# aanna0701/face-recognition-pytorch

Hardware: AMD Instinct MI355X
Metric: train imgs/sec IR-50-layout ResNet50 + ArcFace/PartialFC head, 112x112 (higher is better)
Workload: dtype bf16

## Files before the change

### face-recognition-pytorch_amd/frhip/csrc/bn.hip

```cpp
#include <cstdlib>
#include "common.h"
#include "frhip.h"

namespace frhip {

constexpr int EW_THREADS = 256;
#ifndef EW_UNROLL
#define EW_UNROLL 2
#endif
#ifndef EW_ROWS
#define EW_ROWS 16
#endif
constexpr int RED_GROUPS = 16;

template <typename T> struct EW {
    static constexpr int EPV = 16 / (int)sizeof(T);
};

template <typename T, bool BWD, bool RS = false>
__global__ __launch_bounds__(EW_THREADS) void colreduce_kernel(const T* __restrict__ x, const T* __restrict__ y,
                                                               const float* __restrict__ mean, const float* __restrict__ invstd,
                                                               const float* __restrict__ mscale, const float* __restrict__ mshift,
                                                               float* __restrict__ partial, int rows, int C,
                                                               const float* __restrict__ rowscale = nullptr, int rows_per = 1) {
// ... 116 lines not shown
                                   const float* __restrict__ gamma, const float* __restrict__ beta,
                                   float* __restrict__ running_mean, float* __restrict__ running_var,
                                   float momentum, float eps, float* __restrict__ mean_out,
                                   float* __restrict__ invstd_out, float* __restrict__ scale, float* __restrict__ shift) {
    __shared__ float red[FIN_MAX_PL][2][64];
    int c, pl;
    float s1, s2;
    if constexpr (SMALL) {
        c = blockIdx.x * 16 + (threadIdx.x & 15); pl = threadIdx.x >> 4;
        sum_parts16(parts, nparts, C, c, pl, reinterpret_cast<float (*)[2][16]>(&red[0][0][0]), s1, s2);
    } else {
        c = blockIdx.x * 64 + (threadIdx.x & 63); pl = threadIdx.x >> 6;
        sum_parts(parts, nparts, C, c, pl, red, s1, s2);
    }
    if (pl != 0 || c >= C) return;
    const float mu = s1 / count;
    float var = s2 / count - mu * mu;
    var = var < 0.f ? 0.f : var;
    const float is = rsqrtf(var + eps);
    mean_out[c] = mu; invstd_out[c] = is;
    const float sc = gamma[c] * is;
    scale[c] = sc; shift[c] = beta[c] - mu * sc;
    if (running_mean) {
        running_mean[c] = (1.f - momentum) * running_mean[c] + momentum * mu;
        const float unbiased = count > 1.f ? var * count / (count - 1.f) : var;
        running_var[c] = (1.f - momentum) * running_var[c] + momentum * unbiased;
    }
}

__global__ void bn_eval_kernel(int C, const float* __restrict__ gamma, const float* __restrict__ beta,
                               const float* __restrict__ rm, const float* __restrict__ rv, float eps,
                               float* __restrict__ scale, float* __restrict__ shift) {
    const int c = blockIdx.x * blockDim.x + threadIdx.x;
    if (c >= C) return;
    const float sc = gamma[c] * rsqrtf(rv[c] + eps);
    scale[c] = sc; shift[c] = beta[c] - rm[c] * sc;
}

template <bool SMALL>
__global__ __launch_bounds__(SMALL ? 256 : 1024) void bn_bwd_finalize_kernel(const float* __restrict__ parts, int nparts, int C, float count,
                                       const float* __restrict__ gamma, const float* __restrict__ mean,
                                       const float* __restrict__ invstd, float* __restrict__ dgamma,
                                       float* __restrict__ dbeta, float* __restrict__ ca, float* __restrict__ cb,
                                       float* __restrict__ cc) {
    __shared__ float red[FIN_MAX_PL][2][64];
    int c, pl;
    float s1, s2;
    if constexpr (SMALL) {
        c = blockIdx.x * 16 + (threadIdx.x & 15); pl = threadIdx.x >> 4;
        sum_parts16(parts, nparts, C, c, pl, reinterpret_cast<float (*)[2][16]>(&red[0][0][0]), s1, s2);
    } else {
        c = blockIdx.x * 64 + (threadIdx.x & 63); pl = threadIdx.x >> 6;
        sum_parts(parts, nparts, C, c, pl, red, s1, s2);
    }
    if (pl != 0 || c >= C) return;
    dgamma[c] += s2; dbeta[c] += s1;
    const float gi = gamma[c] * invstd[c], m2 = s2 / count, m1 = s1 / count;
    ca[c] = gi; cb[c] = -gi * invstd[c] * m2; cc[c] = gi * (mean[c] * invstd[c] * m2 - m1);
}

template <typename T, bool NT> __device__ __forceinline__ Vec16<T> ew_load(const T* p) {
    Vec16<T> r;
    if constexpr (NT) r.v = __builtin_nontemporal_load(reinterpret_cast<const decltype(r.v)*>(p));
    else r = *reinterpret_cast<const Vec16<T>*>(p);
    return r;
}
template <typename T, bool NT> __device__ __forceinline__ void ew_store(T* p, const Vec16<T>& x) {
    if constexpr (NT) __builtin_nontemporal_store(x.v, reinterpret_cast<decltype(x.v)*>(p));
    else *reinterpret_cast<Vec16<T>*>(p) = x;
}
static size_t EW_NT_BYTES = (size_t)(getenv("FRHIP_EW_NT_MB") ? atoi(getenv("FRHIP_EW_NT_MB")) : 0) << 20;
static int g_ew_nt = getenv("FRHIP_EW_NT") ? atoi(getenv("FRHIP_EW_NT")) : 1;

template <typename T, bool NTL, bool NTS, bool RS = false, bool INPLACE = false>
__global__ __launch_bounds__(EW_THREADS) void bn_apply_kernel(const T* __restrict__ y_in, const float* __restrict__ scale,
                                                              const float* __restrict__ shift, const T* __restrict__ res,
                                                              const float* __restrict__ rscale, const float* __restrict__ rshift,
                                                              int relu, T* __restrict__ out, int rows, int C,
                                                              const float* __restrict__ rowscale = nullptr, int rows_per = 1) {
    constexpr int EPV = EW<T>::EPV;
    const int vpr = C / EPV;
    const int cg = threadIdx.x % vpr, rl = threadIdx.x / vpr, rlanes = EW_THREADS / vpr;
    float sc[EPV], sh[EPV], rs[EPV], rb[EPV];
    const T* y = INPLACE ? out : y_in;
#pragma unroll
    for (int e = 0; e < EPV; ++e) {
        sc[e] = scale[cg * EPV + e]; sh[e] = shift[cg * EPV + e];
        rs[e] = rscale ? rscale[cg * EPV + e] : 1.f; rb[e] = rscale ? rshift[cg * EPV + e] : 0.f;
    }
#pragma unroll EW_UNROLL
    for (int r = blockIdx.x * rlanes + rl; r < rows; r += gridDim.x * rlanes) {
        const size_t idx = (size_t)r * C + cg * EPV;
        Vec16<T> a = ew_load<T, NTL>(y + idx);
        if constexpr (RS) {
            const float ks = rowscale[r / rows_per];
            Vec16<T> rv;
            if (res) rv = ew_load<T, NTL>(res + idx);
#pragma unroll
            for (int e = 0; e < EPV; ++e) {
                float o = (a.get(e) * sc[e] + sh[e]) * ks + (res ? rv.get(e) * rs[e] + rb[e] : 0.f);
                a.set(e, relu ? fmaxf(o, 0.f) : o);
            }
        } else if (res) {
            const Vec16<T> rv = ew_load<T, NTL>(res + idx);
#pragma unroll
            for (int e = 0; e < EPV; ++e) {
                float o = a.get(e) * sc[e] + sh[e] + (rv.get(e) * rs[e] + rb[e]);
                a.set(e, relu ? fmaxf(o, 0.f) : o);
            }
        } else {
#pragma unroll
            for (int e = 0; e < EPV; ++e) {
                float o = a.get(e) * sc[e] + sh[e];
                a.set(e, relu ? fmaxf(o, 0.f) : o);
            }
        }
        ew_store<T, NTS>(out + idx, a);
    }
}

template <typename T, bool NTL, bool NTS, bool RS = false>
__global__ __launch_bounds__(EW_THREADS) void bn_bwd_apply_kernel(const T* __restrict__ dout, const T* __restrict__ y,
                                                                  const float* __restrict__ ca, const float* __restrict__ cb,
                                                                  const float* __restrict__ cc, const float* __restrict__ mscale,
                                                                  const float* __restrict__ mshift, T* __restrict__ dy,
                                                                  int rows, int C, const float* __restrict__ rowscale = nullptr,
                                                                  int rows_per = 1) {
    constexpr int EPV = EW<T>::EPV;
    const int vpr = C / EPV;
    const int cg = threadIdx.x % vpr, rl = threadIdx.x / vpr, rlanes = EW_THREADS / vpr;
    float a_[EPV], b_[EPV], c_[EPV], ms[EPV], mb[EPV];
#pragma unroll
    for (int e = 0; e < EPV; ++e) {
        a_[e] = ca[cg * EPV + e]; b_[e] = cb[cg * EPV + e]; c_[e] = cc[cg * EPV + e];
        ms[e] = mscale ? mscale[cg * EPV + e] : 0.f; mb[e] = mscale ? mshift[cg * EPV + e] : 1.f;
    }
#pragma unroll EW_UNROLL
    for (int r = blockIdx.x * rlanes + rl; r < rows; r += gridDim.x * rlanes) {
        const size_t idx = (size_t)r * C + cg * EPV;
        const Vec16<T> d = ew_load<T, NTL>(dout + idx);
        Vec16<T> b = ew_load<T, NTL>(y + idx);
        float ks = 1.f;
        if constexpr (RS) ks = rowscale[r / rows_per];
#pragma unroll
        for (int e = 0; e < EPV; ++e) {
            const float yy = b.get(e);
            const float de = (yy * ms[e] + mb[e] > 0.f) ? d.get(e) * ks : 0.f;
            b.set(e, a_[e] * de + b_[e] * yy + c_[e]);
        }
        ew_store<T, NTS>(dy + idx, b);
    }
}

__global__ __launch_bounds__(256) void sum_partials_kernel(const float* __restrict__ partial, int nparts, int C, int which,
                                                           float* __restrict__ out) {
    __shared__ float red[16][16];
    const int cl = threadIdx.x & 15, pl = threadIdx.x >> 4;
    const int c = blockIdx.x * 16 + cl;
    float acc = 0.f;
    if (c < C) {
        int p = pl;
        for (; p + 7 * 16 < nparts; p += 8 * 16) {
            float v[8];
#pragma unroll
            for (int u = 0; u < 8; ++u) v[u] = partial[((size_t)(p + u * 16) * 2 + which) * C + c];
            acc += ((v[0] + v[1]) + (v[2] + v[3])) + ((v[4] + v[5]) + (v[6] + v[7]));
        }
        for (; p < nparts; p += 16) acc += partial[((size_t)p * 2 + which) * C + c];
    }
    red[pl][cl] = acc;
    __syncthreads();
    if (pl == 0 && c < C) {
        float a = 0.f;
#pragma unroll
        for (int l = 0; l < 16; ++l) a += red[l][cl];
        out[c] += a;
    }
}

__global__ void add_bias_kernel(float* __restrict__ x, const float* __restrict__ bias, size_t n, int C) {
    for (size_t i = (size_t)blockIdx.x * blockDim.x + threadIdx.x; i < n; i += (size_t)gridDim.x * blockDim.x)
        x[i] += bias[i % C];
}

template <typename T>
__global__ void cast_from_f32_kernel(const float* __restrict__ src, T* __restrict__ dst, size_t n) {
    for (size_t i = (size_t)blockIdx.x * blockDim.x + threadIdx.x; i < n; i += (size_t)gridDim.x * blockDim.x)
        dst[i] = from_f32<T>(src[i]);
}
template <typename T>
__global__ void cast_to_f32_kernel(const T* __restrict__ src, float* __restrict__ dst, size_t n) {
    for (size_t i = (size_t)blockIdx.x * blockDim.x + threadIdx.x; i < n; i += (size_t)gridDim.x * blockDim.x)
        dst[i] = to_f32<T>(src[i]);
}

static int grid_for(size_t work_items, int per_block) {
    size_t b = (work_items + per_block - 1) / per_block;
    if (b > 2048) b = 2048;
    if (b < 1) b = 1;
    return (int)b;
}

static int ew_row_blocks(int rows, int c, int dtype) {
    const int epv = dtype == FRHIP_DT_BF16 ? 8 : 4;
    const int rlanes = EW_THREADS / (c / epv);
    int b = (rows + rlanes * EW_ROWS - 1) / (rlanes * EW_ROWS);
    if (b > 2048) b = 2048;
    return b < 1 ? 1 : b;
}

static bool shape_ok(int dtype, int C, const char* who) {
    const int epv = dtype == FRHIP_DT_BF16 ? 8 : 4;
    if ((dtype != FRHIP_DT_BF16 && dtype != FRHIP_DT_F32) || C <= 0 || (C % epv) || (C / epv) > EW_THREADS ||
        (EW_THREADS % (C / epv))) {
        set_error("%s: unsupported dtype/channels (dtype=%d C=%d)", who, dtype, C);
        return false;
    }
    return true;
}

}

using namespace frhip;

extern "C" int frhip_colreduce_blocks(int rows, int c, int dtype) {
    const int epv = dtype == FRHIP_DT_BF16 ? 8 : 4;
    if ((dtype != FRHIP_DT_BF16 && dtype != FRHIP_DT_F32) || rows <= 0 || c < epv || (c % epv) || c / epv > EW_THREADS ||
        (EW_THREADS % (c / epv)))
        return 0;
    const int rlanes = EW_THREADS / (c / epv);
    int b = (rows + rlanes * 8 - 1) / (rlanes * 8);
    if (b > 1024) b = 1024;
    if (b < 1) b = 1;
    return b;
}

extern "C" int frhip_colstats(int dtype, const void* x, int rows, int c, float* partial, hipStream_t stream) {
    if (!shape_ok(dtype, c, "frhip_colstats")) return FRHIP_EINVAL;
    const int blocks = frhip_colreduce_blocks(rows, c, dtype);
    if (dtype == FRHIP_DT_BF16)
        hipLaunchKernelGGL((colreduce_kernel<bf16_t, false>), dim3(blocks), dim3(EW_THREADS), 0, stream,
                           (const bf16_t*)x, nullptr, nullptr, nullptr, nullptr, nullptr, partial, rows, c);
    else
        hipLaunchKernelGGL((colreduce_kernel<float, false>), dim3(blocks), dim3(EW_THREADS), 0, stream,
                           (const float*)x, nullptr, nullptr, nullptr, nullptr, nullptr, partial, rows, c);
    return check_launch("frhip_colstats");
}

extern "C" int frhip_bn_bwd_reduce(int dtype, const void* dout, const void* y, const float* mean, const float* invstd,
                                   const float* mask_scale, const float* mask_shift, int rows, int c, float* partial,
                                   hipStream_t stream) {
    if (!shape_ok(dtype, c, "frhip_bn_bwd_reduce")) return FRHIP_EINVAL;
    const int blocks = frhip_colreduce_blocks(rows, c, dtype);
    if (dtype == FRHIP_DT_BF16)
        hipLaunchKernelGGL((colreduce_kernel<bf16_t, true>), dim3(blocks), dim3(EW_THREADS), 0, stream,
                           (const bf16_t*)dout, (const bf16_t*)y, mean, invstd, mask_scale, mask_shift, partial, rows, c);
    else
        hipLaunchKernelGGL((colreduce_kernel<float, true>), dim3(blocks), dim3(EW_THREADS), 0, stream,
                           (const float*)dout, (const float*)y, mean, invstd, mask_scale, mask_shift, partial, rows, c);
    return check_launch("frhip_bn_bwd_reduce");
}

constexpr int FOLD_LIMIT = 512;
static const float* fold_partials(const float* partial, int& nparts, int c, float* scratch, hipStream_t stream) {
    if (nparts <= FOLD_LIMIT) return partial;
    const int groups = 64;
    hipLaunchKernelGGL(reduce_partials_kernel, dim3((2 * c + 63) / 64, groups), dim3(256), 0, stream,
                       partial, scratch, nparts, c);
    nparts = groups;
    return scratch;
}
static int fin_threads(int nparts) { return nparts > 64 ? 1024 : 256; }
static const int g_fin_small = getenv("FRHIP_BN_FIN_SMALL") ? atoi(getenv("FRHIP_BN_FIN_SMALL")) : 1;
static bool fin_small(int nparts) { return g_fin_small == 1 ? nparts > 64 : (g_fin_small >= 2 ? nparts >= g_fin_small : false); }

extern "C" int frhip_bn_finalize(const float* partial, int nparts, float* scratch, int c, float count,
                                 const float* gamma, const float* beta, float* running_mean, float* running_var,
                                 float momentum, float eps, float* mean, float* invstd, float* scale, float* shift,
                                 hipStream_t stream) {
    const float* p = fold_partials(partial, nparts, c, scratch, stream);
    if (fin_small(nparts))
        hipLaunchKernelGGL(bn_finalize_kernel<true>, dim3((c + 15) / 16), dim3(256), 0, stream, p, nparts, c, count, gamma, beta,
                           running_mean, running_var, momentum, eps, mean, invstd, scale, shift);
    else
        hipLaunchKernelGGL(bn_finalize_kernel<false>, dim3((c + 63) / 64), dim3(fin_threads(nparts)), 0, stream, p, nparts, c, count, gamma, beta,
                           running_mean, running_var, momentum, eps, mean, invstd, scale, shift);
    return check_launch("frhip_bn_finalize");
}

extern "C" int frhip_bn_eval_affine(int c, const float* gamma, const float* beta, const float* running_mean,
                                    const float* running_var, float eps, float* scale, float* shift, hipStream_t stream) {
    hipLaunchKernelGGL(bn_eval_kernel, dim3((c + 63) / 64), dim3(64), 0, stream, c, gamma, beta, running_mean,
                       running_var, eps, scale, shift);
    return check_launch("frhip_bn_eval_affine");
}

__global__ void bn_standin_kernel(int c, const float* __restrict__ gamma, const float* __restrict__ beta, float k,
                                  float* __restrict__ mean, float* __restrict__ invstd, float* __restrict__ scale, float* __restrict__ shift) {
    const int i = blockIdx.x * 64 + threadIdx.x;
    if (i >= c) return;
    const float g = gamma[i], b = beta[i], kb = __fmul_rn(k, b);
    const float den = __fadd_rn(__fadd_rn(__fmul_rn(g, g), __fmul_rn(kb, kb)), 1e-20f);
    mean[i] = b; invstd[i] = __fdiv_rn(g, den); scale[i] = 1.f; shift[i] = 0.f;
}
extern "C" int frhip_bn_standin_state(int c, const float* gamma, const float* beta, float k, float* mean, float* invstd,
                                      float* scale, float* shift, hipStream_t stream) {
    if (c <= 0 || !gamma || !beta || !mean || !invstd || !scale || !shift) { frhip::set_error("frhip_bn_standin_state: bad arguments"); return FRHIP_EINVAL; }
    hipLaunchKernelGGL(bn_standin_kernel, dim3((c + 63) / 64), dim3(64), 0, stream, c, gamma, beta, k, mean, invstd, scale, shift);
    return check_launch("frhip_bn_standin_state");
}

extern "C" int frhip_bn_bwd_finalize(const float* partial, int nparts, float* scratch, int c, float count,
                                     const float* gamma, const float* mean, const float* invstd, float* dgamma,
                                     float* dbeta, float* ca, float* cb, float* cc, hipStream_t stream) {
    const float* p = fold_partials(partial, nparts, c, scratch, stream);
    if (fin_small(nparts))
        hipLaunchKernelGGL(bn_bwd_finalize_kernel<true>, dim3((c + 15) / 16), dim3(256), 0, stream, p, nparts, c, count, gamma,
                           mean, invstd, dgamma, dbeta, ca, cb, cc);
    else
        hipLaunchKernelGGL(bn_bwd_finalize_kernel<false>, dim3((c + 63) / 64), dim3(fin_threads(nparts)), 0, stream, p, nparts, c, count, gamma,
                           mean, invstd, dgamma, dbeta, ca, cb, cc);
    return check_launch("frhip_bn_bwd_finalize");
}

extern "C" int frhip_bn_apply_rs(int dtype, const void* y, const float* scale, const float* shift, const void* res,
                                 const float* rowscale, int rows_per, void* out, int rows, int c, hipStream_t stream) {
    if (!shape_ok(dtype, c, "frhip_bn_apply_rs")) return FRHIP_EINVAL;
    if (!rowscale || rows_per <= 0) { set_error("frhip_bn_apply_rs: rowscale and rows_per are required"); return FRHIP_EINVAL; }
    const int blocks = ew_row_blocks(rows, c, dtype);
    if (dtype == FRHIP_DT_BF16)
        hipLaunchKernelGGL((bn_apply_kernel<bf16_t, false, false, true>), dim3(blocks), dim3(EW_THREADS), 0, stream, (const bf16_t*)y, scale,
                           shift, (const bf16_t*)res, nullptr, nullptr, 0, (bf16_t*)out, rows, c, rowscale, rows_per);
    else
        hipLaunchKernelGGL((bn_apply_kernel<float, false, false, true>), dim3(blocks), dim3(EW_THREADS), 0, stream, (const float*)y, scale,
                           shift, (const float*)res, nullptr, nullptr, 0, (float*)out, rows, c, rowscale, rows_per);
    return check_launch("frhip_bn_apply_rs");
}

extern "C" int frhip_bn_bwd_reduce_rs(int dtype, const void* dout, const void* y, const float* mean, const float* invstd,
                                      const float* rowscale, int rows_per, int rows, int c, float* partial, hipStream_t stream) {
    if (!shape_ok(dtype, c, "frhip_bn_bwd_reduce_rs")) return FRHIP_EINVAL;
    if (!rowscale || rows_per <= 0) { set_error("frhip_bn_bwd_reduce_rs: rowscale and rows_per are required"); return FRHIP_EINVAL; }
    const int blocks = frhip_colreduce_blocks(rows, c, dtype);
    if (dtype == FRHIP_DT_BF16)
        hipLaunchKernelGGL((colreduce_kernel<bf16_t, true, true>), dim3(blocks), dim3(EW_THREADS), 0, stream, (const bf16_t*)dout,
                           (const bf16_t*)y, mean, invstd, nullptr, nullptr, partial, rows, c, rowscale, rows_per);
    else
        hipLaunchKernelGGL((colreduce_kernel<float, true, true>), dim3(blocks), dim3(EW_THREADS), 0, stream, (const float*)dout,
                           (const float*)y, mean, invstd, nullptr, nullptr, partial, rows, c, rowscale, rows_per);
    return check_launch("frhip_bn_bwd_reduce_rs");
}

extern "C" int frhip_bn_bwd_apply_rs(int dtype, const void* dout, const void* y, const float* ca, const float* cb, const float* cc,
                                     const float* rowscale, int rows_per, void* dy, int rows, int c, hipStream_t stream) {
    if (!shape_ok(dtype, c, "frhip_bn_bwd_apply_rs")) return FRHIP_EINVAL;
    if (!rowscale || rows_per <= 0) { set_error("frhip_bn_bwd_apply_rs: rowscale and rows_per are required"); return FRHIP_EINVAL; }
    const int blocks = ew_row_blocks(rows, c, dtype);
    if (dtype == FRHIP_DT_BF16)
        hipLaunchKernelGGL((bn_bwd_apply_kernel<bf16_t, false, false, true>), dim3(blocks), dim3(EW_THREADS), 0, stream, (const bf16_t*)dout,
                           (const bf16_t*)y, ca, cb, cc, nullptr, nullptr, (bf16_t*)dy, rows, c, rowscale, rows_per);
    else
        hipLaunchKernelGGL((bn_bwd_apply_kernel<float, false, false, true>), dim3(blocks), dim3(EW_THREADS), 0, stream, (const float*)dout,
                           (const float*)y, ca, cb, cc, nullptr, nullptr, (float*)dy, rows, c, rowscale, rows_per);
    return check_launch("frhip_bn_bwd_apply_rs");
}

extern "C" int frhip_bn_apply(int dtype, const void* y, const float* scale, const float* shift, const void* res,
                              const float* res_scale, const float* res_shift, int relu, void* out, int rows, int c,
                              hipStream_t stream) {
    if (!shape_ok(dtype, c, "frhip_bn_apply")) return FRHIP_EINVAL;
    const int blocks = ew_row_blocks(rows, c, dtype);
    const size_t bytes = (size_t)rows * c * (dtype == FRHIP_DT_BF16 ? 2 : 4);
    const bool ntl = (g_ew_nt & 1) && bytes >= EW_NT_BYTES && (res != nullptr || (g_ew_nt & 4)), nts = (g_ew_nt & 2) && bytes >= EW_NT_BYTES / 2;
#define BN_APPLY_GO(T, L, S)                                                                                                  \
    hipLaunchKernelGGL((bn_apply_kernel<T, L, S>), dim3(blocks), dim3(EW_THREADS), 0, stream, (const T*)y, scale, shift,     \
                       (const T*)res, res_scale, res_shift, relu, (T*)out, rows, c)
#define BN_APPLY_PICK(T)                                                                                                      \
    do { if (ntl && nts) BN_APPLY_GO(T, true, true); else if (ntl) BN_APPLY_GO(T, true, false);                               \
         else if (nts) BN_APPLY_GO(T, false, true); else BN_APPLY_GO(T, false, false); } while (0)
    if (y == out) {
        if (dtype == FRHIP_DT_BF16)
            hipLaunchKernelGGL((bn_apply_kernel<bf16_t, false, false, false, true>), dim3(blocks), dim3(EW_THREADS), 0, stream, nullptr, scale, shift,
                               (const bf16_t*)res, res_scale, res_shift, relu, (bf16_t*)out, rows, c);
        else
            hipLaunchKernelGGL((bn_apply_kernel<float, false, false, false, true>), dim3(blocks), dim3(EW_THREADS), 0, stream, nullptr, scale, shift,
                               (const float*)res, res_scale, res_shift, relu, (float*)out, rows, c);
        return check_launch("frhip_bn_apply");
    }
    if (dtype == FRHIP_DT_BF16) BN_APPLY_PICK(bf16_t); else BN_APPLY_PICK(float);
#undef BN_APPLY_PICK
#undef BN_APPLY_GO
    return check_launch("frhip_bn_apply");
}

extern "C" int frhip_bn_bwd_apply(int dtype, const void* dout, const void* y, const float* ca, const float* cb,
                                  const float* cc, const float* mask_scale, const float* mask_shift, void* dy,
                                  int rows, int c, hipStream_t stream) {
    if (!shape_ok(dtype, c, "frhip_bn_bwd_apply")) return FRHIP_EINVAL;
    const int blocks = ew_row_blocks(rows, c, dtype);
    const size_t bytes = (size_t)rows * c * (dtype == FRHIP_DT_BF16 ? 2 : 4);
    const bool ntl = (g_ew_nt & 1) && bytes >= EW_NT_BYTES, nts = (g_ew_nt & 2) && bytes >= EW_NT_BYTES / 2;
#define BN_BWD_GO(T, L, S)                                                                                                    \
    hipLaunchKernelGGL((bn_bwd_apply_kernel<T, L, S>), dim3(blocks), dim3(EW_THREADS), 0, stream, (const T*)dout, (const T*)y, \
                       ca, cb, cc, mask_scale, mask_shift, (T*)dy, rows, c)
#define BN_BWD_PICK(T)                                                                                                        \
    do { if (ntl && nts) BN_BWD_GO(T, true, true); else if (ntl) BN_BWD_GO(T, true, false);                                   \
         else if (nts) BN_BWD_GO(T, false, true); else BN_BWD_GO(T, false, false); } while (0)
    if (dtype == FRHIP_DT_BF16) BN_BWD_PICK(bf16_t); else BN_BWD_PICK(float);
#undef BN_BWD_PICK
#undef BN_BWD_GO
    return check_launch("frhip_bn_bwd_apply");
}

extern "C" int frhip_sum_partials(const float* partial, int nparts, int c, int which, float* out_accum, hipStream_t stream) {
    hipLaunchKernelGGL(sum_partials_kernel, dim3((c + 15) / 16), dim3(256), 0, stream, partial, nparts, c, which, out_accum);
    return check_launch("frhip_sum_partials");
}

extern "C" int frhip_add_bias(float* x, const float* bias, int rows, int c, hipStream_t stream) {
    const size_t n = (size_t)rows * c;
    hipLaunchKernelGGL(add_bias_kernel, dim3(grid_for(n, 256)), dim3(256), 0, stream, x, bias, n, c);
    return check_launch("frhip_add_bias");
}

extern "C" int frhip_cast_from_f32(int dtype, const float* src, void* dst, size_t n, hipStream_t stream) {
    if (dtype == FRHIP_DT_BF16)
        hipLaunchKernelGGL(cast_from_f32_kernel<bf16_t>, dim3(grid_for(n, 256)), dim3(256), 0, stream, src, (bf16_t*)dst, n);
    else
        hipLaunchKernelGGL(cast_from_f32_kernel<float>, dim3(grid_for(n, 256)), dim3(256), 0, stream, src, (float*)dst, n);
    return check_launch("frhip_cast_from_f32");
}

extern "C" int frhip_cast_to_f32(int dtype, const void* src, float* dst, size_t n, hipStream_t stream) {
    if (dtype == FRHIP_DT_BF16)
        hipLaunchKernelGGL(cast_to_f32_kernel<bf16_t>, dim3(grid_for(n, 256)), dim3(256), 0, stream, (const bf16_t*)src, dst, n);
    else
        hipLaunchKernelGGL(cast_to_f32_kernel<float>, dim3(grid_for(n, 256)), dim3(256), 0, stream, (const float*)src, dst, n);
    return check_launch("frhip_cast_to_f32");
}
```

### include/frhip.h

```cpp
#ifndef FRHIP_H
#define FRHIP_H
#include <stddef.h>
#include <stdint.h>

#ifdef __cplusplus
extern "C" {
#endif

#ifndef FRHIP_STREAM_T
#define FRHIP_STREAM_T
#ifdef __HIP_PLATFORM_AMD__
#include <hip/hip_runtime_api.h>
typedef hipStream_t frhip_stream_t;
#else
typedef void* frhip_stream_t;
#endif
#endif

#define FRHIP_OK 0
#define FRHIP_EINVAL (-1)
#define FRHIP_ELAUNCH (-2)
#define FRHIP_DT_BF16 0
#define FRHIP_DT_F32 1

const char* frhip_last_error(void);
int frhip_abi_version(void);
int frhip_spin(long long ticks, frhip_stream_t stream);

int frhip_nt_block_m(int k);
int frhip_conv_stat_rows(int dtype, int m, int k, int h, int w, int c, int r, int s, int stride, int pad);
int frhip_set_wgrad_taps9(int enabled);
int frhip_set_conv_halo(int enabled);
int frhip_set_halo_wide_dirs(int dirs);
int frhip_set_epi_lean(int enabled);
int frhip_set_nt_tile(int tile);
int frhip_conv_fwd_affine(int dtype, const void* x, const void* w, void* y, const float* scale, const float* shift, int relu,
                          const void* residual, int n, int h, int wd, int c, int k, int r, int s, int stride, int pad,
                          frhip_stream_t stream);
int frhip_conv_fwd(int dtype, const void* x, const void* w, void* y, float* stats_partial,
                   int n, int h, int wd, int c, int k, int r, int s, int stride, int pad, frhip_stream_t stream);
int frhip_conv_dgrad(int dtype, const void* dy, const void* wt, void* dx, const void* residual,
                     int n, int h, int wd, int c, int k, int r, int s, int stride, int pad, frhip_stream_t stream);
int frhip_dgrad_stat_rows(int dtype, int n, int h, int wd, int c, int k, int r, int s, int stride, int pad);
int frhip_conv_dgrad_bnred(int dtype, const void* dy, const void* wt, void* dx, const void* residual,
                           const void* y_bn, const float* mean, const float* invstd, const float* mask_scale,
                           const float* mask_shift, float* stats_partial, int n, int h, int wd, int c, int k,
                           int r, int s, int stride, int pad, frhip_stream_t stream);
int frhip_conv_dgrad_fused(int dtype, const void* dy, const void* wt, void* dx, const void* residual, int residual_stride,
                           const void* y_bn, const float* mean, const float* invstd, const float* mask_scale,
                           const float* mask_shift, float* stats_partial, int n, int h, int wd, int c, int k,
                           int r, int s, int stride, int pad, frhip_stream_t stream);
int frhip_conv_dgrad_fused_rs(int dtype, const void* dy, const void* wt, void* dx, const void* residual, int residual_stride,
                              const void* y_bn, const float* mean, const float* invstd, const float* mask_scale,
                              const float* mask_shift, const float* rowscale, int rows_per, float keep_scale,
                              float* stats_partial, int n, int h, int wd, int c, int k, int r, int s, int stride, int pad,
                              frhip_stream_t stream);
int frhip_conv_wgrad(int dtype, const void* dy, const void* x, float* dw, int n, int h, int w, int c,
                     int k, int r, int s, int stride, int pad, int splits, float* workspace, size_t workspace_bytes,
                     frhip_stream_t stream);
int frhip_conv_wgrad_chain_ok(int dtype, int n, int h, int w, int c, int k, int r, int s, int stride, int pad);
int frhip_conv_wgrad_chain(int dtype, const void* dy, const void* x, int n, int h, int w, int c, int k, float* slabs,
                           size_t slab_bytes, float* prev_dw, const float* prev_slabs, int prev_k, int prev_c, int prev_splits,
                           int* splits_out, frhip_stream_t stream);
int frhip_conv_wgrad_chain_finish(float* dw, float* slabs, int k, int c, int splits, frhip_stream_t stream);
int frhip_linear_fwd(int dtype, const void* a, const void* w, const float* bias, void* out, void* act_out,
                     float* stats_partial, int m, int n, int k, frhip_stream_t stream);
int frhip_linear_dgrad_gelu(int dtype, const void* dy, const void* wt, const void* pre, void* dx, float* stats_partial,
                            int m, int n, int k, frhip_stream_t stream);
int frhip_gemm_nt(int dtype, const void* a, const void* b, void* out, int m, int n, int k, int splits,
                  int atomic_f32, frhip_stream_t stream);
int frhip_gemm_nt_splitk(int dtype, const void* a, const void* b, const float* bias, float* out, int m, int n, int k,
                         int splits, float* slabs, size_t slab_bytes, frhip_stream_t stream);
int frhip_gemm_tn(int dtype, const void* p, const void* q, float* out, int m, int kc, int ldp, int c,
                  int splits, float* workspace, size_t workspace_bytes, frhip_stream_t stream);
int frhip_gemm_tn_overwrite(int dtype, const void* p, const void* q, float* out, int m, int kc, int ldp, int c,
                            float* workspace, size_t workspace_bytes, frhip_stream_t stream);

int frhip_colreduce_blocks(int rows, int c, int dtype);
int frhip_colstats(int dtype, const void* x, int rows, int c, float* partial, frhip_stream_t stream);
int frhip_bn_finalize(const float* partial, int nparts, float* scratch, int c, float count,
                      const float* gamma, const float* beta, float* running_mean, float* running_var,
                      float momentum, float eps, float* mean, float* invstd, float* scale, float* shift,
                      frhip_stream_t stream);
int frhip_bn_eval_affine(int c, const float* gamma, const float* beta, const float* running_mean,
                         const float* running_var, float eps, float* scale, float* shift, frhip_stream_t stream);
int frhip_bn_standin_state(int c, const float* gamma, const float* beta, float k, float* mean, float* invstd, float* scale,
                           float* shift, frhip_stream_t stream);
int frhip_bn_apply(int dtype, const void* y, const float* scale, const float* shift, const void* res,
                   const float* res_scale, const float* res_shift, int relu, void* out, int rows, int c,
                   frhip_stream_t stream);
int frhip_bn_bwd_reduce(int dtype, const void* dout, const void* y, const float* mean, const float* invstd,
                        const float* mask_scale, const float* mask_shift, int rows, int c, float* partial,
                        frhip_stream_t stream);
int frhip_bn_bwd_finalize(const float* partial, int nparts, float* scratch, int c, float count,
                          const float* gamma, const float* mean, const float* invstd, float* dgamma,
                          float* dbeta, float* ca, float* cb, float* cc, frhip_stream_t stream);
int frhip_bn_bwd_apply(int dtype, const void* dout, const void* y, const float* ca, const float* cb,
                       const float* cc, const float* mask_scale, const float* mask_shift, void* dy,
                       int rows, int c, frhip_stream_t stream);
int frhip_bn_apply_rs(int dtype, const void* y, const float* scale, const float* shift, const void* res, const float* rowscale,
                      int rows_per, void* out, int rows, int c, frhip_stream_t stream);
int frhip_bn_bwd_reduce_rs(int dtype, const void* dout, const void* y, const float* mean, const float* invstd, const float* rowscale,
                           int rows_per, int rows, int c, float* partial, frhip_stream_t stream);
int frhip_bn_bwd_apply_rs(int dtype, const void* dout, const void* y, const float* ca, const float* cb, const float* cc,
                          const float* rowscale, int rows_per, void* dy, int rows, int c, frhip_stream_t stream);
int frhip_sum_partials(const float* partial, int nparts, int c, int which, float* out_accum, frhip_stream_t stream);
int frhip_add_bias(float* x, const float* bias, int rows, int c, frhip_stream_t stream);
int frhip_cast_from_f32(int dtype, const float* src, void* dst, size_t n, frhip_stream_t stream);
int frhip_cast_to_f32(int dtype, const void* src, float* dst, size_t n, frhip_stream_t stream);

int frhip_stem_im2col(int dtype, const float* x, void* col, int b, int h, int w, int stride, frhip_stream_t stream);
int frhip_bn_relu_maxpool_fwd(int dtype, const void* y, const float* scale, const float* shift, void* out,
                              uint8_t* argmax, int b, int h, int w, int c, frhip_stream_t stream);
int frhip_maxpool_bwd(int dtype, const void* dpool, const uint8_t* argmax, void* da, int b, int h, int w,
                      int c, frhip_stream_t stream);

int frhip_pack_wt(int dtype, const float* w, void* wt, int k, int rs, int c, frhip_stream_t stream);
int frhip_transpose2d(int dtype_in, int dtype_out, const void* in, void* out, int rows, int cols, int ld_out,
                      frhip_stream_t stream);
int frhip_pack_stem(int dtype, const float* w, void* wp, int k, int kin, int kp, frhip_stream_t stream);
int frhip_unpack_stem_grad(const float* dwp, float* dw, int k, int kin, int kp, frhip_stream_t stream);
int frhip_fc_permute(int dtype, const float* w, void* wp, int nout, int c, int hw, frhip_stream_t stream);
int frhip_fc_unpermute_grad(const float* dwp, float* dw, int nout, int c, int hw, frhip_stream_t stream);
int frhip_pfc_sample_max_local(void);
int frhip_pfc_sample(const int64_t* labels, int n, long long class_start, int num_local, const float* u, int num_sample,
                     int64_t* index_out, int* rel_out, int64_t* n_positive, frhip_stream_t stream);
int frhip_gather_rows(const float* src, const int64_t* index, float* dst, int n, int d, frhip_stream_t stream);
int frhip_scatter_rows(const float* src, const int64_t* index, float* dst, int n, int d, frhip_stream_t stream);

int frhip_head_dw_ok(int dtype, int n, int classes, int d);
int frhip_head_dw(int dtype, const void* dt, int ldt, const void* ehat, const void* what, const float* wnorm, float* dw,
                  int n, int classes, int d, float out_scale, frhip_stream_t stream);
int frhip_l2norm_rows(int dtype, const float* x, void* xhat, float* norms, int rows, int d, float eps,
                      frhip_stream_t stream);
int frhip_l2norm_bwd(int dtype, const float* dxhat, const void* xhat, const float* norms, float* dx,
                     int rows, int d, float out_scale, frhip_stream_t stream);
int frhip_head_groups(int num_classes);
int frhip_head_fwd(int dtype, const void* ehat, const void* what, const int* labels, int n, int classes,
                   int d, float s, float m, float* part_max, float* part_sum, float* ztarget,
                   float* rowmax, float* rowsum, frhip_stream_t stream);
int frhip_head_rescale(float* rowsum, const float* local_max, const float* global_max, int n, frhip_stream_t stream);
int frhip_head_target_prob(const float* ztarget, const int* labels, const float* rowmax, const float* rowsum,
                           float* q, int n, frhip_stream_t stream);
int frhip_head_pack_stats(const float* ztarget, const int* labels, const float* rowmax, const float* rowsum,
                          float* packed, int n, frhip_stream_t stream);
int frhip_head_merge_stats(const float* gathered, int world_size, int n, float* rowmax, float* rowsum, float* q,
                           frhip_stream_t stream);
int frhip_head_loss(const float* q, int n, float* loss, frhip_stream_t stream);
int frhip_head_bwd_dt(int dtype, const void* ehat, const void* what, const int* labels, int n, int classes,
                      int d, float s, float m, const float* rowmax, const float* rowsum, float gscale,
                      const float* upstream, void* dt, int ldt, void* dtt, int ldtt, frhip_stream_t stream);

int frhip_conv_bnrelu_fusable(int dtype, int h, int wd, int c, int k, int r, int s, int stride, int pad);
int frhip_conv_fwd_bnrelu(int dtype, const void* x, const float* in_scale, const float* in_shift, const void* w, void* y,
                          float* stats_partial, void* act_out, int n, int h, int wd, int c, int k, int r, int s, int stride,
                          int pad, frhip_stream_t stream);
int frhip_conv_wgrad_bnrelu_fusable(int dtype, int n, int h, int w, int c, int k, int r, int s, int stride, int pad);
int frhip_conv_wgrad_bnrelu(int dtype, const void* dy, const void* x, const float* in_scale, const float* in_shift,
                            float* dw, int n, int h, int w, int c, int k, int r, int s, int stride, int pad, int splits,
                            float* workspace, size_t workspace_bytes, frhip_stream_t stream);

int frhip_quant_fp8_weights(const float* w, void* w8, float* scale, int k, int rowlen, frhip_stream_t stream);
typedef struct { const float* w; void* w8; float* scale; int32_t k, rowlen, row_begin, pad_; } frhip_q8w;
int frhip_quant_fp8_weights_multi(const frhip_q8w* table, int ntensors, int nrows, frhip_stream_t stream);
int frhip_fp8_saturation(int op);
int frhip_quant_fp8(int dtype, const void* x, void* x8, size_t n, float inv_scale, frhip_stream_t stream);
int frhip_bn_apply_q8(int dtype, const void* y, const float* scale, const float* shift, const void* res,
                      const float* res_scale, const float* res_shift, int relu, void* out, void* out8, float inv_q,
                      int rows, int c, frhip_stream_t stream);
int frhip_conv_fwd_fp8(const void* x8, const void* w8, const float* wscale, float act_scale, void* y,
                       float* stats_partial, int n, int h, int wd, int c, int k, int r, int s, int stride, int pad,
                       frhip_stream_t stream);
int frhip_fp8_stat_rows(int m, int k);
int frhip_fp8_conv_stat_rows(int m, int k, int h, int w, int c, int r, int s, int stride, int pad);
int frhip_set_fp8_halo(int enabled);
int frhip_linear_fwd_fp8(const void* a8, const void* w8, const float* wscale, float act_scale, const float* bias,
                         void* out, float* stats_partial, int m, int n, int k, frhip_stream_t stream);

typedef struct frhip_cpb_block {
    const void* coords;
    const void* index;
    const void* w0;
    const void* b0;
    const void* w2;
    const void* logit_scale;
    void* bias;
    void* scale;
// ... 98 lines not shown
```

Before: 22070.

## Add software-pipelined streaming BN apply kernels with LDS coefficients and CU-sized grids

Adds streaming variants of the BN forward-apply and backward-apply elementwise kernels. Each workgroup owns a contiguous row range sized so the grid matches the CU count, stages per-channel coefficients in LDS, and double-buffers batches of 4 rows so loads of the next batch overlap compute and stores of the current one. The new path is on by default behind FRHIP_EW_STREAM and a setter. It raises register pressure, and the clamped tail loads are redundant.

Result: faster. 22620 (median of 6 runs) (+2.5%).

```diff
diff --git a/face-recognition-pytorch_amd/frhip/csrc/bn.hip b/face-recognition-pytorch_amd/frhip/csrc/bn.hip
--- a/face-recognition-pytorch_amd/frhip/csrc/bn.hip
+++ b/face-recognition-pytorch_amd/frhip/csrc/bn.hip
@@ -292,6 +292,129 @@
     }
 }
 
+constexpr int ST_R = 4;
+
+template <typename T, bool HAS_RES, bool RS>
+struct ApplyOp {
+    static constexpr int NIN = HAS_RES ? 2 : 1, NCOEF = HAS_RES ? 4 : 2;
+    int relu;
+    __device__ __forceinline__ void operator()(Vec16<T>* u, const f32x4_t* k, float ks, int e0) const {
+        Vec16<T>& a = u[0];
+#pragma unroll
+        for (int i = 0; i < 4; ++i) {
+            const int e = e0 + i;
+            float o;
+            if constexpr (RS) o = (a.get(e) * k[0][i] + k[1][i]) * ks + (HAS_RES ? u[NIN - 1].get(e) * k[NCOEF - 2][i] + k[NCOEF - 1][i] : 0.f);
+            else if constexpr (HAS_RES) o = a.get(e) * k[0][i] + k[1][i] + (u[1].get(e) * k[2][i] + k[3][i]);
+            else o = a.get(e) * k[0][i] + k[1][i];
+            a.set(e, relu ? fmaxf(o, 0.f) : o);
+        }
+    }
+};
+template <typename T, bool RS>
+struct BwdApplyOp {
+    static constexpr int NIN = 2, NCOEF = 5;
+    __device__ __forceinline__ void operator()(Vec16<T>* u, const f32x4_t* k, float ks, int e0) const {
+        const Vec16<T>& d = u[0];
+        Vec16<T>& b = u[1];
+#pragma unroll
+        for (int i = 0; i < 4; ++i) {
+            const int e = e0 + i;
+            const float yy = b.get(e);
+            const float de = (yy * k[3][i] + k[4][i] > 0.f) ? d.get(e) * ks : 0.f;
+            b.set(e, k[0][i] * de + k[1][i] * yy + k[2][i]);
+        }
+    }
+};
+
+template <typename T, int NIN, bool RS>
+struct StBatch {
+    Vec16<T> u[ST_R][NIN];
+    float ks[ST_R];
+};
+template <typename T, int NIN, bool NTL, bool RS>
+__device__ __forceinline__ void st_load(StBatch<T, NIN, RS>& b, const T* const* in, int r, int step, int rlast, int C, int col,
+                                        const float* __restrict__ rowscale, int rows_per) {
+#pragma unroll
+    for (int j = 0; j < ST_R; ++j) {
+        const int rr = min(r + j * step, rlast);
+        const size_t idx = (size_t)rr * C + col;
+#pragma unroll
+        for (int i = 0; i < NIN; ++i) b.u[j][i] = ew_load<T, NTL>(in[i] + idx);
+        if constexpr (RS) b.ks[j] = rowscale[rr / rows_per];
+        else b.ks[j] = 1.f;
+    }
+}
+template <typename T, int NIN, bool NTS, bool RS, int OUT_IN, class Op>
+__device__ __forceinline__ void st_compute_store(StBatch<T, NIN, RS>& b, const Op& op, const float* lds, int r, int step, int rend, int C,
+                                                 int col, T* __restrict__ out) {
+    constexpr int EPV = EW<T>::EPV;
+#pragma unroll
+    for (int e0 = 0; e0 < EPV; e0 += 4) {
+        f32x4_t k[Op::NCOEF];
+#pragma unroll
+        for (int q = 0; q < Op::NCOEF; ++q) k[q] = *reinterpret_cast<const f32x4_t*>(lds + q * C + col + e0);
+#pragma unroll
+        for (int j = 0; j < ST_R; ++j) op(b.u[j], k, b.ks[j], e0);
+    }
+#pragma unroll
+    for (int j = 0; j < ST_R; ++j) {
+        const int rr = r + j * step;
+        if (rr < rend) ew_store<T, NTS>(out + (size_t)rr * C + col, b.u[j][OUT_IN]);
+    }
+}
+
+template <typename T, bool NTL, bool NTS, bool RS, int OUT_IN, class Op>
+__device__ __forceinline__ void ew_stream(const Op& op, const T* const* in, const float* const* coef, const float* cdef, T* out,
+                                          int rows, int C, int rows_wg, const float* __restrict__ rowscale, int rows_per) {
+    constexpr int EPV = EW<T>::EPV, NIN = Op::NIN;
+    extern __shared__ float st_lds[];
+    const int vpr = C / EPV;
+    const int col = (threadIdx.x % vpr) * EPV, rl = threadIdx.x / vpr, rlanes = EW_THREADS / vpr;
+    const int r0 = blockIdx.x * rows_wg, rend = min(rows, r0 + rows_wg), rlast = rend - 1;
+    const int bstep = rlanes * ST_R;
+    const int nb = (rend - r0 - rl + bstep - 1) / bstep;
+    StBatch<T, NIN, RS> A, B;
+    st_load<T, NIN, NTL, RS>(A, in, r0 + rl, rlanes, rlast, C, col, rowscale, rows_per);
+#pragma unroll
+    for (int q = 0; q < Op::NCOEF; ++q)
+        for (int c = threadIdx.x; c < C; c += EW_THREADS) st_lds[q * C + c] = coef[q] ? coef[q][c] : cdef[q];
+    __syncthreads();
+    for (int b = 0; b < nb; b += 2) {
+        const int ra = r0 + rl + b * bstep;
+        st_load<T, NIN, NTL, RS>(B, in, ra + bstep, rlanes, rlast, C, col, rowscale, rows_per);
+        st_compute_store<T, NIN, NTS, RS, OUT_IN>(A, op, st_lds, ra, rlanes, rend, C, col, out);
+        if (b + 1 >= nb) break;
+        st_load<T, NIN, NTL, RS>(A, in, ra + 2 * bstep, rlanes, rlast, C, col, rowscale, rows_per);
+        st_compute_store<T, NIN, NTS, RS, OUT_IN>(B, op, st_lds, ra + bstep, rlanes, rend, C, col, out);
+    }
+}
+
+template <typename T, bool NTL, bool NTS, bool HAS_RES, bool RS = false, bool INPLACE = false>
+__global__ __launch_bounds__(EW_THREADS) void bn_apply_stream_kernel(const T* __restrict__ y_in, const float* __restrict__ scale,
+                                                                     const float* __restrict__ shift, const T* __restrict__ res,
+                                                                     const float* __restrict__ rscale, const float* __restrict__ rshift,
+                                                                     int relu, T* __restrict__ out, int rows, int C, int rows_wg,
+                                                                     const float* __restrict__ rowscale = nullptr, int rows_per = 1) {
+    const T* in[2] = {INPLACE ? out : y_in, res};
+    const float* coef[4] = {scale, shift, rscale, rscale ? rshift : nullptr};
+    const float cdef[4] = {0.f, 0.f, 1.f, 0.f};
+    ew_stream<T, NTL, NTS, RS, 0>(ApplyOp<T, HAS_RES, RS>{relu}, in, coef, cdef, out, rows, C, rows_wg, rowscale, rows_per);
+}
+
+template <typename T, bool NTL, bool NTS, bool RS = false>
+__global__ __launch_bounds__(EW_THREADS) void bn_bwd_apply_stream_kernel(const T* __restrict__ dout, const T* __restrict__ y,
+                                                                         const float* __restrict__ ca, const float* __restrict__ cb,
+                                                                         const float* __restrict__ cc, const float* __restrict__ mscale,
+                                                                         const float* __restrict__ mshift, T* __restrict__ dy,
+                                                                         int rows, int C, int rows_wg,
+                                                                         const float* __restrict__ rowscale = nullptr, int rows_per = 1) {
+    const T* in[2] = {dout, y};
+    const float* coef[5] = {ca, cb, cc, mscale, mscale ? mshift : nullptr};
+    const float cdef[5] = {0.f, 0.f, 0.f, 0.f, 1.f};
+    ew_stream<T, NTL, NTS, RS, 1>(BwdApplyOp<T, RS>{}, in, coef, cdef, dy, rows, C, rows_wg, rowscale, rows_per);
+}
+
 __global__ __launch_bounds__(256) void sum_partials_kernel(const float* __restrict__ partial, int nparts, int C, int which,
                                                            float* __restrict__ out) {
     __shared__ float red[16][16];
@@ -349,6 +472,28 @@
     return b < 1 ? 1 : b;
 }
 
+static int g_ew_stream = getenv("FRHIP_EW_STREAM") ? atoi(getenv("FRHIP_EW_STREAM")) : 1;
+static const int g_ew_stream_wgs = getenv("FRHIP_EW_STREAM_WGS") ? atoi(getenv("FRHIP_EW_STREAM_WGS")) : 1;
+static int ew_cus() {
+    static int cus[16] = {0};
+    int dev = 0;
+    if (hipGetDevice(&dev) != hipSuccess || dev < 0 || dev >= 16) { (void)hipGetLastError(); return 256; }
+    if (!cus[dev]) {
+        int v = 0;
+        if (hipDeviceGetAttribute(&v, hipDeviceAttributeMultiprocessorCount, dev) != hipSuccess || v <= 0) v = 256;
+        cus[dev] = v;
+    }
+    return cus[dev];
+}
+static int ew_stream_blocks(int rows, int c, int dtype, int& rows_wg) {
+    const int epv = dtype == FRHIP_DT_BF16 ? 8 : 4;
+    const int bstep = EW_THREADS / (c / epv) * ST_R;
+    const long long steps = (rows + bstep - 1) / bstep, target = (long long)ew_cus() * (g_ew_stream_wgs > 0 ? g_ew_stream_wgs : 1);
+    const long long per = (steps + target - 1) / target;
+    rows_wg = (int)(per * bstep);
+    return (int)((rows + rows_wg - 1) / rows_wg);
+}
+
 static bool shape_ok(int dtype, int C, const char* who) {
     const int epv = dtype == FRHIP_DT_BF16 ? 8 : 4;
     if ((dtype != FRHIP_DT_BF16 && dtype != FRHIP_DT_F32) || C <= 0 || (C % epv) || (C / epv) > EW_THREADS ||
@@ -467,6 +612,18 @@
                                  const float* rowscale, int rows_per, void* out, int rows, int c, hipStream_t stream) {
     if (!shape_ok(dtype, c, "frhip_bn_apply_rs")) return FRHIP_EINVAL;
     if (!rowscale || rows_per <= 0) { set_error("frhip_bn_apply_rs: rowscale and rows_per are required"); return FRHIP_EINVAL; }
+    if (g_ew_stream) {
+        int rwg = 0;
+        const int blocks = ew_stream_blocks(rows, c, dtype, rwg);
+#define BN_APPLY_RS_GO(T, R)                                                                                                  \
+        hipLaunchKernelGGL((bn_apply_stream_kernel<T, false, false, R, true>), dim3(blocks), dim3(EW_THREADS),              \
+                           (R ? 4 : 2) * c * sizeof(float), stream, (const T*)y, scale, shift, (const T*)res, nullptr, nullptr, 0, \
+                           (T*)out, rows, c, rwg, rowscale, rows_per)
+        if (dtype == FRHIP_DT_BF16) { if (res) BN_APPLY_RS_GO(bf16_t, true); else BN_APPLY_RS_GO(bf16_t, false); }
+        else { if (res) BN_APPLY_RS_GO(float, true); else BN_APPLY_RS_GO(float, false); }
+#undef BN_APPLY_RS_GO
+        return check_launch("frhip_bn_apply_rs");
+    }
     const int blocks = ew_row_blocks(rows, c, dtype);
     if (dtype == FRHIP_DT_BF16)
         hipLaunchKernelGGL((bn_apply_kernel<bf16_t, false, false, true>), dim3(blocks), dim3(EW_THREADS), 0, stream, (const bf16_t*)y, scale,
@@ -495,6 +652,17 @@
                                      const float* rowscale, int rows_per, void* dy, int rows, int c, hipStream_t stream) {
     if (!shape_ok(dtype, c, "frhip_bn_bwd_apply_rs")) return FRHIP_EINVAL;
     if (!rowscale || rows_per <= 0) { set_error("frhip_bn_bwd_apply_rs: rowscale and rows_per are required"); return FRHIP_EINVAL; }
+    if (g_ew_stream) {
+        int rwg = 0;
+        const int blocks = ew_stream_blocks(rows, c, dtype, rwg);
+        if (dtype == FRHIP_DT_BF16)
+            hipLaunchKernelGGL((bn_bwd_apply_stream_kernel<bf16_t, false, false, true>), dim3(blocks), dim3(EW_THREADS), 5 * c * sizeof(float),
+                               stream, (const bf16_t*)dout, (const bf16_t*)y, ca, cb, cc, nullptr, nullptr, (bf16_t*)dy, rows, c, rwg, rowscale, rows_per);
+        else
+            hipLaunchKernelGGL((bn_bwd_apply_stream_kernel<float, false, false, true>), dim3(blocks), dim3(EW_THREADS), 5 * c * sizeof(float),
+                               stream, (const float*)dout, (const float*)y, ca, cb, cc, nullptr, nullptr, (float*)dy, rows, c, rwg, rowscale, rows_per);
+        return check_launch("frhip_bn_bwd_apply_rs");
+    }
     const int blocks = ew_row_blocks(rows, c, dtype);
     if (dtype == FRHIP_DT_BF16)
         hipLaunchKernelGGL((bn_bwd_apply_kernel<bf16_t, false, false, true>), dim3(blocks), dim3(EW_THREADS), 0, stream, (const bf16_t*)dout,
@@ -509,9 +677,27 @@
                               const float* res_scale, const float* res_shift, int relu, void* out, int rows, int c,
                               hipStream_t stream) {
     if (!shape_ok(dtype, c, "frhip_bn_apply")) return FRHIP_EINVAL;
-    const int blocks = ew_row_blocks(rows, c, dtype);
     const size_t bytes = (size_t)rows * c * (dtype == FRHIP_DT_BF16 ? 2 : 4);
     const bool ntl = (g_ew_nt & 1) && bytes >= EW_NT_BYTES && (res != nullptr || (g_ew_nt & 4)), nts = (g_ew_nt & 2) && bytes >= EW_NT_BYTES / 2;
+    if (g_ew_stream) {
+        int rwg = 0;
+        const int blocks = ew_stream_blocks(rows, c, dtype, rwg);
+#define BN_ST_GO(T, L, S, R, IP)                                                                                              \
+        hipLaunchKernelGGL((bn_apply_stream_kernel<T, L, S, R, false, IP>), dim3(blocks), dim3(EW_THREADS),                 \
+                           (R ? 4 : 2) * c * sizeof(float), stream, IP ? nullptr : (const T*)y, scale, shift, (const T*)res,    \
+                           res_scale, res_shift, relu, (T*)out, rows, c, rwg)
+#define BN_ST_RES(T, L, S) do { if (res) BN_ST_GO(T, L, S, true, false); else BN_ST_GO(T, L, S, false, false); } while (0)
+#define BN_ST_PICK(T)                                                                                                         \
+        do { if (y == out) { if (res) BN_ST_GO(T, false, false, true, true); else BN_ST_GO(T, false, false, false, true); }   \
+             else if (ntl && nts) BN_ST_RES(T, true, true); else if (ntl) BN_ST_RES(T, true, false);                         \
+             else if (nts) BN_ST_RES(T, false, true); else BN_ST_RES(T, false, false); } while (0)
+        if (dtype == FRHIP_DT_BF16) BN_ST_PICK(bf16_t); else BN_ST_PICK(float);
+#undef BN_ST_PICK
+#undef BN_ST_RES
+#undef BN_ST_GO
+        return check_launch("frhip_bn_apply");
+    }
+    const int blocks = ew_row_blocks(rows, c, dtype);
 #define BN_APPLY_GO(T, L, S)                                                                                                  \
     hipLaunchKernelGGL((bn_apply_kernel<T, L, S>), dim3(blocks), dim3(EW_THREADS), 0, stream, (const T*)y, scale, shift,     \
                        (const T*)res, res_scale, res_shift, relu, (T*)out, rows, c)
@@ -537,9 +723,23 @@
                                   const float* cc, const float* mask_scale, const float* mask_shift, void* dy,
                                   int rows, int c, hipStream_t stream) {
     if (!shape_ok(dtype, c, "frhip_bn_bwd_apply")) return FRHIP_EINVAL;
-    const int blocks = ew_row_blocks(rows, c, dtype);
     const size_t bytes = (size_t)rows * c * (dtype == FRHIP_DT_BF16 ? 2 : 4);
     const bool ntl = (g_ew_nt & 1) && bytes >= EW_NT_BYTES, nts = (g_ew_nt & 2) && bytes >= EW_NT_BYTES / 2;
+    if (g_ew_stream) {
+        int rwg = 0;
+        const int blocks = ew_stream_blocks(rows, c, dtype, rwg);
+#define BN_BWD_ST_GO(T, L, S)                                                                                                 \
+        hipLaunchKernelGGL((bn_bwd_apply_stream_kernel<T, L, S>), dim3(blocks), dim3(EW_THREADS), 5 * c * sizeof(float), stream, \
+                           (const T*)dout, (const T*)y, ca, cb, cc, mask_scale, mask_shift, (T*)dy, rows, c, rwg)
+#define BN_BWD_ST_PICK(T)                                                                                                     \
+        do { if (ntl && nts) BN_BWD_ST_GO(T, true, true); else if (ntl) BN_BWD_ST_GO(T, true, false);                       \
+             else if (nts) BN_BWD_ST_GO(T, false, true); else BN_BWD_ST_GO(T, false, false); } while (0)
+        if (dtype == FRHIP_DT_BF16) BN_BWD_ST_PICK(bf16_t); else BN_BWD_ST_PICK(float);
+#undef BN_BWD_ST_PICK
+#undef BN_BWD_ST_GO
+        return check_launch("frhip_bn_bwd_apply");
+    }
+    const int blocks = ew_row_blocks(rows, c, dtype);
 #define BN_BWD_GO(T, L, S)                                                                                                    \
     hipLaunchKernelGGL((bn_bwd_apply_kernel<T, L, S>), dim3(blocks), dim3(EW_THREADS), 0, stream, (const T*)dout, (const T*)y, \
                        ca, cb, cc, mask_scale, mask_shift, (T*)dy, rows, c)
@@ -552,6 +752,12 @@
     return check_launch("frhip_bn_bwd_apply");
 }
 
+extern "C" int frhip_set_ew_stream(int enabled) {
+    const int old = g_ew_stream;
+    if (enabled >= 0) g_ew_stream = enabled != 0;
+    return old;
+}
+
 extern "C" int frhip_sum_partials(const float* partial, int nparts, int c, int which, float* out_accum, hipStream_t stream) {
     hipLaunchKernelGGL(sum_partials_kernel, dim3((c + 15) / 16), dim3(256), 0, stream, partial, nparts, c, which, out_accum);
     return check_launch("frhip_sum_partials");
diff --git a/include/frhip.h b/include/frhip.h
--- a/include/frhip.h
+++ b/include/frhip.h
@@ -33,6 +33,7 @@
 int frhip_set_conv_halo(int enabled);
 int frhip_set_halo_wide_dirs(int dirs);
 int frhip_set_epi_lean(int enabled);
+int frhip_set_ew_stream(int enabled);
 int frhip_set_nt_tile(int tile);
 int frhip_conv_fwd_affine(int dtype, const void* x, const void* w, void* y, const float* scale, const float* shift, int relu,
                           const void* residual, int n, int h, int wd, int c, int k, int r, int s, int stride, int pad,
```
